# puzzlepaint/camera_calibration

Measured on AMD Instinct MI355X. Metric: M observations/sec per LM iteration, higher is better.
Workload: dtype f64

## Files before the change

camera_calibration_amd/build.py:

```python
from __future__ import annotations

import os
import shutil
import subprocess
import sys

HERE = os.path.dirname(os.path.abspath(__file__))
CSRC = os.path.join(HERE, "csrc")
LIB = os.path.join(HERE, "libcalib_ba_hip.so")
SOURCES = ["cba_api.hip", "cba_setup.hip", "cba_passes.hip", "cba_solve.hip", "cba_posefirst.hip", "cba_gridfirst.hip", "cba_oneshot.hip", "cba_report.hip", "cba_compare.hip", "cba_undistort.hip", "cba_features.hip",
           "kernels_project.hip", "kernels_fd.hip", "kernels_obs.hip", "kernels_update.hip", "kernels_linalg.hip", "kernels_ldlt.hip", "kernels_ldlt_dist.hip", "kernels_backsolve.hip", "kernels_fit.hip", "gridfirst_plan.hip", "kernels_gridfirst.hip", "kernels_report.hip", "kernels_compare.hip", "kernels_undistort.hip", "kernels_features.hip", "cba_localize.hip", "kernels_localize.hip", "cba_localize_images.hip", "kernels_localize_images.hip", "cba_parametric.hip", "kernels_parametric.hip", "cba_stereo.hip", "kernels_stereo.hip", "kernels_stereo_post.hip"]
HEADERS = ["cba_internal.h", "hip_buf.h", "cba_problem.h", "cba_model.h", "model.hip.h", "obs_device.hip.h", "block_device.hip.h", "localize_device.hip.h", "gridfirst_plan.h", "linalg_internal.h", "ldlt_dataflow.hip.h", os.path.join("..", "..", "include", "cba.h")]
PUBLIC_HEADERS = [os.path.join("..", "..", "include", "cba_undistort.h"), os.path.join("..", "..", "include", "cba_features.h"),
                  os.path.join("..", "..", "include", "cba_stereo.h"), os.path.join("..", "..", "include", "cba_stereo_post.h"),
                  os.path.join("..", "..", "include", "cba_diagnostics.h")]
FLAGS = ["--offload-arch=gfx950", "-O3", "-std=c++17", "-fPIC", "-munsafe-fp-atomics", "-Wall", "-Wno-unused-function", "-Wno-unused-value", "-Wno-unused-result",
         "-mllvm", "-amdgpu-mfma-vgpr-form"]


def _hipcc() -> str:
    for cand in (shutil.which("hipcc"), "/opt/rocm/bin/hipcc"):
        if cand and os.path.exists(cand):
            return cand
    raise RuntimeError("hipcc not found")


FLAGS_STAMP = os.path.join(HERE, ".build_flags")
# ... 222 lines not shown
```

camera_calibration_amd/csrc/cba_api.hip:

```cpp
#include <algorithm>
#include <cmath>
#include <cstdlib>
#include <cstring>
#include <memory>

#include "cba_problem.h"
#include "../../include/cba_diagnostics.h"

namespace cba {

static thread_local std::string g_error;
void set_error(const std::string& msg) { g_error = msg; }

struct GpermView { int* v[kMaxCameras] = {}; };
static GpermView gperm_view(const cba_problem* p) {
  GpermView g;
  for (int c = 0; c < kMaxCameras; ++c) g.v[c] = p->gperm[c];
  return g;
}

static int enqueue_candidate_cost(cba_problem* p, int cand, const int* guard) {
  CBA_TRY(launch_apply_update(p->L, p->cams, p->st[p->cur], p->x, p->st[cand], p->pose_slot, gperm_view(p).v, p->stream));
  CBA_TRY(residual_pass(p, cand, guard));
  return launch_reduce_costs(p->out.cost_ref, p->out.cost_test, nullptr, p->obs.n, p->red_partials, p->red8, p->stream);
// ... 51 lines not shown
  setenv("GPU_MAX_HW_QUEUES", "8", 0);
  CBA_TRY(select_device(config->device, "cba_create: "));
  std::unique_ptr<cba_problem, decltype(&cba_destroy)> p(new cba_problem(), &cba_destroy);
  p->cfg = *config;
  p->cams.assign(config->cameras, config->cameras + config->n_cameras);
  p->cfg.cameras = p->cams.data();
  p->device = config->device;
  make_layout(p->cfg, p->L);
  if (p->L.total_dof <= 0) { set_error("empty problem"); return CBA_ERR_ARG; }
  CBA_TRY(make_main_stream(&p->stream));
  CBA_TRY(choose_elimination_order(p.get(), config));
  CBA_TRY(alloc_pass_buffers(p.get()));
  CBA_TRY(alloc_system(p.get()));
  CBA_TRY(alloc_reduce_buffer(p.get(), config));
  CBA_TRY(setup_gf_sharding(p.get()));
  CBA_TRY(alloc_ldlt_workspace(p.get()));
  *out = p.release();
  return CBA_OK;
}

void cba_destroy(cba_problem* p) {
  if (!p) return;
  hipSetDevice(p->device);
  if (p->stream) hipStreamSynchronize(p->stream);
  delete p;
}

int cba_set_observations(cba_problem* p, int64_t n, const float* xy, const int32_t* point_index,
                         const int32_t* image_index, const int32_t* camera_index, const double* last_projection) {
  if (!p || n < 0 || (n > 0 && (!xy || !point_index || !image_index || !camera_index))) { set_error("cba_set_observations: bad argument"); return CBA_ERR_ARG; }
// ... 408 lines not shown
  for (int i = 0; i < 3; ++i) out[i] = v[i];
  return CBA_OK;
}
int cba_debug_straggler_stats(cba_problem* p, int64_t out[5]) {
  if (!p || !out || !p->slow.count) { set_error("cba_debug_straggler_stats: bad argument"); return CBA_ERR_ARG; }
  int v[kSlowCounters];
  CBA_HIP(hipSetDevice(p->device));
  CBA_HIP(hipStreamSynchronize(p->stream));
  CBA_TRY(p->slow.count.download(v, kSlowCounters));
  out[0] = 0;
  out[1] = v[kSlowListCount] < p->slow.cap ? v[kSlowListCount] : p->slow.cap;
  out[2] = v[kSlowStatPeriod1]; out[3] = v[kSlowStatPeriodN]; out[4] = v[kSlowStatFullBudget];
  return CBA_OK;
}

}
```

camera_calibration_amd/csrc/cba_internal.h:

```cpp
#pragma once
#include <hip/hip_runtime.h>
#include <stdint.h>

#include <chrono>
#include <string>
#include <type_traits>
#include <vector>

#include "../../include/cba.h"
#include "../../include/cba_features.h"
#include "gridfirst_plan.h"
#include "hip_buf.h"
#include "model.hip.h"

namespace cba {

class Event {
 public:
  Event() = default;
  Event(Event&& o) noexcept : e_(o.e_) { o.e_ = nullptr; }
  Event& operator=(Event&& o) noexcept {
    if (this != &o) { reset(); e_ = o.e_; o.e_ = nullptr; }
    return *this;
  }
// ... 150 lines not shown
                      const double* det_scale, int points_separate, hipStream_t s);
int launch_accumulate_points(const PassArgs& a, const Layout& L, const std::vector<cba_camera>& cams, const Observations& obs,
                             const PassOutputs& out, const SystemView& sys, const double* det_scale, hipStream_t s);
int launch_det_scale(const PassArgs& a, const PassOutputs& out, DetMode& det, hipStream_t s);
int launch_det_convert(double* p, size_t n, const double* det_scale, hipStream_t s);
int launch_accumulate_strips(const PassArgs& a, const Layout& L, const Observations& obs, const PassOutputs& out, CellSort& cell,
                             const SystemView& sys, const double* det_scale, hipStream_t s);
int launch_accumulate_cells(const PassArgs& a, const std::vector<cba_camera>& cams, const PassOutputs& out, CellSort& cell,
                            const SystemView& sys, int rig_row_first, const double* det_scale, hipStream_t s);
int launch_exclusive_scan(const int* count, int n, int* start, hipStream_t s);
int launch_reduce_costs(const double* ref, const double* test, const uint8_t* flags, int64_t n, double* partials,
                        double* out8, hipStream_t s);
int launch_apply_update(const Layout& L, const std::vector<cba_camera>& cams, const DevState& in, const double* x,
                        DevState& out, const int* pose_slot, int* const* gperm, hipStream_t s);
int launch_update_direction_grid(const double* in, const double* x, int G, double* out, hipStream_t s);
int launch_fit_pass(bool jac, int gw, int gh, const double* grid, const double* tang, int64_t n, const double* gp,
                    const double* dirs, double* cost_vec, double* rec, int* keys, int* status, hipStream_t s);
int launch_fit_accumulate(int gw, int gh, int64_t n, const double* rec, const int* keys, DevBuf<int>& count, int* start, DevBuf<int>& fill,
                          int* order, double* H, int ld, double* b, hipStream_t s);
int launch_fit_set_rhs(double* S, int ld, const double* b, int n, hipStream_t s);
int launch_fit_diag_sum(const double* H, int ld, int n, double* out, hipStream_t s);

int launch_direction_image(const CamDev* cam_dev, int model, int W, int H, double* dirs, uint8_t* ok, uint8_t* rgb, hipStream_t s,
                           bool use_stage = true);
struct SiteGrid {
  int side4;
  int bw, bh;
  const int* start;
  const int* order;
  const int* xy;
// ... 264 lines not shown
```

camera_calibration_amd/csrc/cba_passes.hip:

```cpp
#include "cba_problem.h"

namespace cba {

int timer_begin(cba_problem* p, int which, hipStream_t s) {
  KernelTimer& t = p->timers[which];
  if (t.used == (int)t.spans.size()) {
    KernelTimer::Span sp;
    CBA_TRY(sp.e0.create()); CBA_TRY(sp.e1.create());
    t.spans.push_back(std::move(sp));
  }
  CBA_HIP(hipEventRecord(t.spans[t.used].e0, s ? s : p->stream));
  return CBA_OK;
}
int timer_end(cba_problem* p, int which, double flops, double bytes, int launches, hipStream_t s) {
  KernelTimer& t = p->timers[which];
  CBA_HIP(hipEventRecord(t.spans[t.used].e1, s ? s : p->stream));
  t.used += 1;
  t.flops += flops; t.bytes += bytes; t.launches += launches;
  return CBA_OK;
}
int timers_collect(cba_problem* p) {
  for (KernelTimer& t : p->timers) {
    for (int i = 0; i < t.used; ++i) {
      CBA_HIP(hipEventSynchronize(t.spans[i].e1));
// ... 63 lines not shown
  CBA_HIP(hipEventRecord(p->ev_aux2, p->stream));
  CBA_HIP(hipStreamWaitEvent(aux, p->ev_aux2, 0));
  CBA_TRY(launch_base_project_slow(as, p->model_mask, p->out,  false, p->slow, aux));
  CBA_TRY(launch_fd_tasks(as, p->model_mask, L.localize_only, p->out, p->fd, kFdSideList, aux));
  CBA_HIP(hipEventRecord(p->ev_aux1, aux));
  CBA_TRY(timer_begin(p, kTimerFd));
  CBA_TRY(launch_fd_tasks(a, p->model_mask, L.localize_only, p->out, p->fd, kFdMainList, p->stream));
  CBA_TRY(timer_end(p, kTimerFd, 0, 0, 1));
  CBA_HIP(hipStreamWaitEvent(clr, p->ev_aux2, 0));
  CBA_TRY(p->sys.Dblk.zero_async(clr));
  CBA_TRY(p->sys.bblk.zero_async(clr));
  if (L.eliminate_points)
    CBA_TRY(p->sys.B.zero_async(clr));
  else
    CBA_TRY(p->sys.B.zero_async((size_t)(p->sys.Kpad - L.block_dof) * p->sys.n_pad, clr, (size_t)L.block_dof * p->sys.n_pad));
  CBA_TRY(p->sys.Hdd.zero_async(clr));
  CBA_TRY(p->sys.bd.zero_async(clr));
  if (p->gf.S0) CBA_TRY(p->gf.S0.zero_async(clr));
  CBA_HIP(hipEventRecord(p->ev_clear, clr));
  CBA_HIP(hipStreamWaitEvent(p->stream, p->ev_aux1, 0));
  CBA_HIP(hipStreamWaitEvent(p->stream, p->ev_clear, 0));
  a.skip = nullptr;
  const bool side = !L.localize_only;
  CBA_TRY(launch_assemble(a, L, p->st[w], p->out, p->slow, p->stream));
  double t0 = now_s();
  CBA_TRY(timer_begin(p, kTimerAccumulate));
  SystemView T = p->sys.view();
  const double* det = p->cfg.deterministic ? (const double*)p->det.scale : nullptr;
  if (det) CBA_TRY(launch_det_scale(a, p->out, p->det, p->stream));
  const int points_separate = (!L.eliminate_points && p->obs.pt_start) ? 1 : 0;
  if (p->gf.S0) {
// ... 5 lines not shown
    CBA_HIP(hipStreamWaitEvent(aux, p->ev_aux0, 0));
    CBA_TRY(launch_accumulate_cells(a, p->cams, p->out, p->cell, T, (!L.eliminate_points && L.rig_in_state) ? L.first_camera_tr_rig - L.block_dof : -1,
                                    det, aux));
    if (p->gridfirst) CBA_TRY(gridfirst_pass_activity(p, a, aux));
    CBA_HIP(hipEventRecord(p->ev_aux1, aux));
  }
  if (points_separate)
    CBA_TRY(launch_accumulate_points(a, L, p->cams, p->obs, p->out, T, det, p->stream));
  if (!L.eliminate_points)
    CBA_TRY(launch_accumulate_strips(a, L, p->obs, p->out, p->cell, T, det, p->stream));
  CBA_TRY(launch_accumulate(a, L, p->out, p->cell, T, det, points_separate, p->stream));
  if (side) CBA_HIP(hipStreamWaitEvent(p->stream, p->ev_aux1, 0));
  if (det) {
    CBA_TRY(launch_det_convert(p->sys.Dblk, nb * bs * bs, det, p->stream));
    CBA_TRY(launch_det_convert(p->sys.bblk, nb * bs, det + 1, p->stream));
    CBA_TRY(launch_det_convert(p->sys.Hdd, (size_t)L.dense_dof * p->sys.n_pad, det, p->stream));
    CBA_TRY(launch_det_convert(p->sys.bd, (size_t)p->sys.n_pad, det + 1, p->stream));
    CBA_TRY(launch_det_convert(p->sys.B, (size_t)L.block_dof * p->sys.n_pad, det, p->stream));
    if (p->gf.S0) CBA_TRY(launch_det_convert(p->gf.S0, p->gf.S0.size(), det, p->stream));
  }
  CBA_TRY(timer_end(p, kTimerAccumulate, 0, 0, 1));
  if (t_acc) *t_acc += now_s() - t0;
  CBA_TRY(p->gridfirst ? gridfirst_pass_end(p) : posefirst_pass_end(p));
  p->have_system = true;
  return CBA_OK;
}

}
```

camera_calibration_amd/csrc/cba_problem.h:

```cpp
#pragma once
#include <cmath>

#include "cba_internal.h"

using namespace cba;

struct KernelTimer {
  struct Span { Event e0, e1; };
  std::vector<Span> spans;
  int used = 0;
  double seconds = 0, flops = 0, bytes = 0;
  int launches = 0;
};
enum Timer {
  kTimerProduct,
  kTimerFactor,
  kTimerAccumulate,
  kTimerFd,
  kTimerFactorGemm,
  kTimerJacobianPass,
  kTimerSolve,
  kTimerCost,
  kNumTimers
};
// ... 19 lines not shown
  PinnedBuf<unsigned long long> kmask_host;
  double update_flops = 0;
  DevBuf<int> tile_list; PinnedBuf<int> tile_list_host; bool tile_list_valid = false; unsigned tile_list_age = 0;
  int tile_list_entries = 0;
  bool tile_list_dirty = false;
};

struct GfShardState {
  GfShared shared;
  DevBuf<int> shared_col;
  int rank = 0, world = 1, img0 = 0, max_local = 0;
  std::vector<int> counts, offsets;
  DevBuf<double> gDblk, gbblk, gB;
  DevBuf<double> gsend, grecv; int64_t gblk = 0;
};
#pragma GCC visibility pop

struct cba_problem {
  cba_config cfg{};
  std::vector<cba_camera> cams;
  Layout L{};
  int device = 0;
  hipStream_t stream = nullptr;
  bool have_obs = false, have_state = false, have_system = false;
  int model_mask = 0;
  Observations obs;
  PassOutputs out;
  StragglerSplit slow;
  FdWork fd;
  CellSort cell;
  DetMode det;
  DevState st[2];
  int cur = 0;
  DevBuf<double> itg;
  DevBuf<double> tangents[kMaxCameras];
  DevBuf<CamDev> cams_dev[2];
  std::vector<int> pose_slot_host; DevBuf<int> pose_slot;
  Event ev_aux0, ev_aux1, ev_aux2, ev_clear;
  DevBuf<int> gperm[kMaxCameras];
  std::vector<int> dense_perm_host;
  DevBuf<double> red_partials, red8;
  NormalSystem sys;
  double* P = nullptr; DevBuf<double> P_own;
  DevBuf<double> P2;
  int64_t P_cap = 0;
  DevBuf<double> x, scal;
  DevBuf<int> status;
  LdltWorkspace ldlt;
  KernelTimer timers[kNumTimers];
  double last_lambda = 0;
  PinnedBuf<double> pin_status;
  PinnedBuf<double> pin_cost;
  double last_x0 = 0;
  bool gridfirst = false;
  bool gf_sharded = false;
  PoseFirstState pf;
  GridFirstState gf;
// ... 15 lines not shown
      if (cx < 0 || cy < 0 || cx >= cm.grid_w || cy >= cm.grid_h) continue;
      fn(cx, cy);
    }
}
inline int common_slabs(const unsigned long long* a, const unsigned long long* b, int words) {
  int n = 0;
  for (int w = 0; w < words; ++w) n += __builtin_popcountll(a[w] & b[w]);
  return n;
}

void make_layout(const cba_config& cfg, Layout& L);
int check_config(const cba_config* config);
int choose_elimination_order(cba_problem* p, const cba_config* config);
int alloc_pass_buffers(cba_problem* p);
int alloc_system(cba_problem* p);
int alloc_reduce_buffer(cba_problem* p, const cba_config* config);
int alloc_ldlt_workspace(cba_problem* p);
void order_imagesets(cba_problem* p, int64_t n, const float* xy, const int32_t* point_index, const int32_t* image_index,
                     const int32_t* camera_index, std::vector<int>& order);

int timer_begin(cba_problem* p, int which, hipStream_t s = nullptr);
int timer_end(cba_problem* p, int which, double flops, double bytes, int launches, hipStream_t s = nullptr);
int timers_collect(cba_problem* p);
int allreduce(cba_problem* p, double* dev, int64_t count);
int residual_pass(cba_problem* p, int which, const int* guard = nullptr);
int jacobian_pass_and_accumulate(cba_problem* p, double* t_acc);

int solve_enqueue(cba_problem* p, double lambda);
int solve_finish(cba_problem* p);
int solve_system(cba_problem* p, double lambda);
// ... 21 lines not shown
```

camera_calibration_amd/csrc/cba_setup.hip:

```cpp
#include <algorithm>
#include <map>
#include <mutex>

#include "cba_problem.h"

namespace cba {

void make_layout(const cba_config& cfg, Layout& L) {
  L.n_cameras = cfg.n_cameras; L.n_images = cfg.n_images; L.n_points = cfg.n_points;
  L.localize_only = cfg.localize_only ? 1 : 0;
  L.eliminate_points = cfg.eliminate_points ? 1 : 0;
  const int N = cfg.n_images, C = cfg.n_cameras, P = cfg.n_points;
  L.rig_in_state = C > 1;
  const int rig_dof = L.rig_in_state ? 6 * C : 0;
  L.first_rig_tr_global = L.eliminate_points ? 3 * P : 0;
  L.first_camera_tr_rig = L.first_rig_tr_global + 6 * N;
  L.first_points = L.eliminate_points ? 0 : L.first_camera_tr_rig + rig_dof;
  L.first_intrinsics = L.eliminate_points ? (L.first_camera_tr_rig + rig_dof) : (L.first_points + 3 * P);
  if (L.eliminate_points) { L.block_size = 3; L.n_blocks = P; } else { L.block_size = 6; L.n_blocks = N; }
  L.block_dof = L.block_size * L.n_blocks;
  int off = L.first_intrinsics;
  for (int c = 0; c < C; ++c) {
    L.intr_offset[c] = off - L.block_dof;
    off += unknowns_per_point(cfg.cameras[c].model_type) * cfg.cameras[c].grid_w * cfg.cameras[c].grid_h;
// ... 76 lines not shown
  if (o->factor_tail_rows > 0) w.tail_rows = o->factor_tail_rows;
  w.back_dataflow = o->back_substitution == 0;
}

static int alloc_state(cba_problem* p, DevState& s) {
  CBA_TRY(s.rig_tr_global.alloc(7 * (size_t)p->L.n_images));
  CBA_TRY(s.camera_tr_rig.alloc(7 * (size_t)p->L.n_cameras));
  CBA_TRY(s.points.alloc(3 * (size_t)p->L.n_points));
  for (int c = 0; c < p->L.n_cameras; ++c) {
    size_t G = (size_t)p->cams[c].grid_w * p->cams[c].grid_h;
    CBA_TRY(s.grids[c].alloc(doubles_per_point(p->cams[c].model_type) * G));
  }
  return CBA_OK;
}

static int build_grid_order(cba_problem* p) {
  const Layout& L = p->L;
  p->dense_perm_host.resize(L.dense_dof);
  for (int i = 0; i < L.dense_dof; ++i) p->dense_perm_host[i] = i;
  if (L.localize_only) return CBA_OK;
  for (int c = 0; c < L.n_cameras; ++c) {
    const int gw = p->cams[c].grid_w, gh = p->cams[c].grid_h;
    const int per = unknowns_per_point(p->cams[c].model_type);
    const int tile = per == 2 ? 8 : 5;
    std::vector<int> perm((size_t)gw * gh);
    int rank = 0;
    if (p->gridfirst) perm = p->gf.plan.gperm[c];
    else
    for (int ty = 0; ty < gh; ty += tile)
      for (int tx = 0; tx < gw; tx += tile)
        for (int y = ty; y < std::min(gh, ty + tile); ++y)
          for (int x = tx; x < std::min(gw, tx + tile); ++x) perm[x + (size_t)y * gw] = rank++;
    CBA_TRY(p->gperm[c].assign(perm));
    for (size_t g = 0; g < perm.size(); ++g)
      for (int d = 0; d < per; ++d)
        p->dense_perm_host[L.intr_offset[c] + per * g + d] = L.intr_offset[c] + per * perm[g] + d;
  }
  return CBA_OK;
}

static int upload_camdevs(cba_problem* p, int which) {
  std::vector<CamDev> h(p->L.n_cameras);
  for (int c = 0; c < p->L.n_cameras; ++c)
    h[c] = make_camdev(p->cams[c], p->st[which].grids[c], p->tangents[c], p->L.intr_offset[c], p->gperm[c]);
  CBA_TRY(p->cams_dev[which].upload_async(h.data(), h.size(), p->stream));
  CBA_HIP(hipStreamSynchronize(p->stream));
  return CBA_OK;
}

int check_config(const cba_config* config) {
  if (!config || !config->cameras || config->n_cameras < 1 || config->n_cameras > kMaxCameras ||
      config->n_images < 0 || config->n_points < 0 || !(config->numerical_diff_delta > 0)) {
// ... 102 lines not shown
  CBA_TRY(p->det.bits.alloc(2)); CBA_TRY(p->det.scale.alloc(2));
  CBA_TRY(p->fd.redo_count.alloc_zero(4));
  CBA_TRY(p->red_partials.alloc(256 * 8));
  CBA_TRY(p->red8.alloc(16));
  return CBA_OK;
}

int alloc_system(cba_problem* p) {
  const Layout& L = p->L;
  padded_dims(L.dense_dof, &p->sys.n_pad, &p->sys.n_fact);
  p->sys.Kpad = round_up(L.block_dof > 0 ? L.block_dof : 1, 48);
  const size_t bs = L.block_size, nb = L.n_blocks;
  CBA_TRY(p->sys.Dblk.alloc(nb * bs * bs));
  CBA_TRY(p->sys.bblk.alloc(nb * bs));
  CBA_TRY(p->sys.B.alloc((size_t)p->sys.Kpad * p->sys.n_pad));
  CBA_TRY(p->sys.Hdd.alloc((size_t)p->sys.n_pad * p->sys.n_pad));
  CBA_TRY(p->sys.bd.alloc((size_t)p->sys.n_pad));
  CBA_TRY(p->gridfirst ? alloc_gridfirst_system(p) : alloc_posefirst_system(p));
  CBA_TRY(p->x.alloc_zero((size_t)L.block_dof + p->sys.n_pad));
  CBA_TRY(p->scal.alloc(16));
  CBA_TRY(p->status.alloc(2));
  CBA_TRY(p->pin_status.alloc(4));
  CBA_TRY(p->pin_cost.alloc(16));
  return CBA_OK;
}

int alloc_reduce_buffer(cba_problem* p, const cba_config* config) {
  if (!config->allreduce) return CBA_OK;
  int64_t need = p->gf_sharded ? p->sh.shared.doubles : packed_upper_doubles(p->sys.n_pad);
  if (config->distributed_solve) {
    need = (int64_t)ldlt_dist_buffer_doubles(p->sys.n_pad, config->world_size);
// ... 47 lines not shown
```

camera_calibration_amd/csrc/kernels_update.hip:

```cpp
#include "block_device.hip.h"
#include "obs_device.hip.h"

namespace cba {

constexpr int kRedBlocks = 256;
__global__ void __launch_bounds__(256) k_reduce_costs_partial(const double* __restrict__ ref, const double* __restrict__ test,
                                                              const uint8_t* __restrict__ flags, int64_t n,
                                                              double* __restrict__ partials) {
  double acc[8] = {0, 0, 0, 0, 0, 0, 0, 0};
  for (int64_t i = (int64_t)blockIdx.x * 256 + threadIdx.x; i < n; i += (int64_t)kRedBlocks * 256) {
    double r = ref ? ref[i] : -1.0, t = test ? test[i] : -1.0;
    if (r >= 0) { acc[0] += r; acc[5] += 1; }
    if (t >= 0) { acc[1] += t; acc[6] += 1; }
    if (r >= 0 && t >= 0) { acc[2] += r; acc[3] += t; acc[4] += 1; }
    if (flags && flags[i] == 1) acc[7] += 1;
  }
  __shared__ double sh[8][256];
  block_reduce_256(acc, sh, SumOp());
  if (threadIdx.x < 8) partials[blockIdx.x * 8 + threadIdx.x] = sh[threadIdx.x][0];
}
int launch_reduce_costs(const double* ref, const double* test, const uint8_t* flags, int64_t n, double* partials,
                        double* out8, hipStream_t s) {
  hipLaunchKernelGGL(k_reduce_costs_partial, dim3(kRedBlocks), dim3(256), 0, s, ref, test, flags, n, partials);
  hipLaunchKernelGGL((k_fold_partials<8, kRedBlocks, SumOp>), dim3(1), dim3(64), 0, s, partials, out8);
// ... 73 lines not shown
    hipLaunchKernelGGL(k_update_grid, dim3((G + 255) / 256), dim3(256), 0, s, in.grids[c],
                       x + (L.localize_only ? 0 : L.block_dof + L.intr_offset[c]), G, per, L.localize_only ? 0 : 1,
                       gperm ? gperm[c] : nullptr, out.grids[c]);
  }
  CBA_HIP(hipGetLastError());
  return CBA_OK;
}

int launch_update_direction_grid(const double* in, const double* x, int G, double* out, hipStream_t s) {
  if (G == 0) return CBA_OK;
  hipLaunchKernelGGL(k_update_grid, dim3((G + 255) / 256), dim3(256), 0, s, in, x, G, 2, 1, (const int*)nullptr, out);
  CBA_HIP(hipGetLastError());
  return CBA_OK;
}

}
```

camera_calibration_amd/engine.py:

```python
from __future__ import annotations

import ctypes as C
import os
from dataclasses import dataclass
from typing import Callable, List, Optional, Sequence

import numpy as np

from .problem import CENTRAL_GENERIC, Camera, Problem, State

_HERE = os.path.dirname(os.path.abspath(__file__))
LIB_PATH = os.environ.get("CBA_HIP_LIB") or os.path.join(_HERE, "libcalib_ba_hip.so")


class EngineError(RuntimeError):
    pass


class CbaCamera(C.Structure):
    _fields_ = [("model_type", C.c_int32), ("width", C.c_int32), ("height", C.c_int32),
                ("calib_min_x", C.c_int32), ("calib_min_y", C.c_int32),
                ("calib_max_x", C.c_int32), ("calib_max_y", C.c_int32),
                ("grid_w", C.c_int32), ("grid_h", C.c_int32)]

# ... 202 lines not shown
    "cba_remap_apply_device": (_I, [_VP, _I32, _I32, _I32, _I32, _VP, _VP, C.c_uint8, _VP]),
}


class CbaStereoOptions(C.Structure):
    _fields_ = [("context_radius", C.c_int32), ("iterations", C.c_int32), ("min_depth", C.c_float), ("max_depth", C.c_float),
                ("max_normal_2d_length", C.c_float), ("cost_threshold", C.c_float), ("angle_threshold", C.c_float),
                ("lr_consistency_factor_threshold", C.c_float), ("seed", C.c_uint64)]


_I8P, _SOPT = C.POINTER(C.c_int8), C.POINTER(CbaStereoOptions)
DIAGNOSTICS_PROTOTYPES = {
    "cba_debug_straggler_stats": (_I, [_VP, _I64P]),
    "cba_debug_gridfirst_tile_list_query": (_I64, [_I32, _I32, _I32, C.POINTER(C.c_uint64), _I32, _I32, _I32P, _I64]),
    "cba_debug_gridfirst_tile_list": (_I64, [_VP, _I32P, _I64, _I32P]),
}
STEREO_PROTOTYPES = {
    "cba_stereo_create": (_I, [_I32, _I32, _I32, _I32, _F32P, C.c_float, C.c_float, C.c_float, C.c_float, _I32, _I32, _F32P, _F32P, _I32,
                               C.POINTER(_VP)]),
    "cba_stereo_destroy": (None, [_VP]),
    "cba_stereo_set_images": (_I, [_VP, _U8, _U8]),
    "cba_stereo_set_pose": (_I, [_VP, _F32P]),
    "cba_stereo_match": (_I, [_VP, _SOPT]),
    "cba_stereo_get_state": (_I, [_VP, _F32P, _I8P, _F32P]),
    "cba_stereo_set_state": (_I, [_VP, _F32P, _I8P, _F32P]),
    "cba_stereo_run_stage": (_I, [_VP, _SOPT, _I32, _I32]),
    "cba_stereo_cost": (_I, [_VP, _SOPT, _F32P, _I8P, _F32P]),
    "cba_stereo_filter": (_I, [_VP, _SOPT, _F32P, _F32P]),
}
STEREO_INIT, STEREO_MUTATION, STEREO_PROPAGATION, STEREO_REFINEMENT = 0, 1, 2, 3
# ... 26 lines not shown
def load() -> C.CDLL:
    global _lib
    if _lib is not None:
        return _lib
    os.environ.setdefault("GPU_MAX_HW_QUEUES", "8")
    try:
        import torch
    except Exception:
        pass
    if not os.path.exists(LIB_PATH):
        raise EngineError(f"{LIB_PATH} is missing -- run `python -c 'import __graft_entry__ as g; g.build()'`; "
                          "the engine has no CPU fallback")
    L = C.CDLL(LIB_PATH)
    for name, (restype, argtypes) in {**PROTOTYPES, **UNDISTORT_PROTOTYPES, **STEREO_PROTOTYPES, **STEREO_POST_PROTOTYPES,
                                      **DIAGNOSTICS_PROTOTYPES}.items():
        fn = getattr(L, name)
        fn.restype, fn.argtypes = restype, argtypes
    _lib = L
    return L


def gridfirst_plan(cameras: Sequence[Camera], n_images: int, n_points: int, strips: int = 0, single_tile_tasks: bool = False) -> dict:
    L = load()
    cams = (CbaCamera * len(cameras))(*[_cam_struct(c) for c in cameras])

    def q(what, dtype):
        n = L.cba_gridfirst_plan_query(cams, len(cameras), n_images, n_points, strips, int(single_tile_tasks), what, None, 0)
        if n < 0:
            _check(int(n), "cba_gridfirst_plan_query")
        out = np.zeros(int(n) // np.dtype(dtype).itemsize, dtype=dtype)
        if n:
# ... 19 lines not shown

def gridfirst_tile_list_query(mode: int, masks: np.ndarray, n_slabs: int, allow_parts: bool) -> np.ndarray:
    L = load()
    m = np.ascontiguousarray(masks, dtype=np.uint64)
    assert m.ndim == 2
    mp = m.ctypes.data_as(C.POINTER(C.c_uint64))
    n = int(L.cba_debug_gridfirst_tile_list_query(int(mode), m.shape[0], m.shape[1], mp, int(n_slabs), int(bool(allow_parts)), None, 0))
    if n < 0:
        _check(n, "cba_debug_gridfirst_tile_list_query")
    out = np.zeros((n, 4), dtype=np.int32)
    if n:
        got = int(L.cba_debug_gridfirst_tile_list_query(int(mode), m.shape[0], m.shape[1], mp, int(n_slabs), int(bool(allow_parts)),
                                                        out.ctypes.data_as(_I32P), n))
        assert got == n
    return out


def prepare(device: int = 0) -> None:
    _check(load().cba_prepare_device(int(device)), "cba_prepare_device")


def _check(rc: int, what: str) -> None:
    if rc != 0:
        msg = load().cba_last_error()
        raise EngineError(f"{what} failed with code {rc}: {msg.decode() if msg else ''}")


def _dp(a: np.ndarray):
    assert a.dtype == np.float64 and a.flags.c_contiguous
    return a.ctypes.data_as(C.POINTER(C.c_double))
# ... 157 lines not shown
    def straggler_stats(self) -> dict:
        out = (C.c_int64 * 5)()
        _check(self.L.cba_debug_straggler_stats(self._h, out), "cba_debug_straggler_stats")
        return dict(zip(("predicted", "listed", "period_1", "period_2_or_more", "full_budget"), (int(v) for v in out)))

    def gridfirst_tile_list(self):
        info = (C.c_int32 * 4)()
        n = int(self.L.cba_debug_gridfirst_tile_list(self._h, None, 0, info))
        if n < 0:
            _check(n, "cba_debug_gridfirst_tile_list")
        out = np.zeros((n, 4), dtype=np.int32)
        if n:
            assert int(self.L.cba_debug_gridfirst_tile_list(self._h, out.ctypes.data_as(_I32P), n, info)) == n
        return out, dict(valid=int(info[0]), age=int(info[1]), dirty=int(info[2]), n_slabs=int(info[3]))

    def debug_accumulate(self) -> float:
        cost = C.c_double(0)
        _check(self.L.cba_debug_accumulate(self._h, C.byref(cost)), "cba_debug_accumulate")
        return cost.value

    def debug_solve(self, lam: float) -> np.ndarray:
        _check(self.L.cba_debug_solve(self._h, lam), "cba_debug_solve")
        return self.dump(DUMP_X)

    def debug_apply_update(self, x: np.ndarray) -> None:
        x = np.ascontiguousarray(x, dtype=np.float64)
        assert x.size == self.problem.total_dof
        _check(self.L.cba_debug_apply_update(self._h, _dp(x)), "cba_debug_apply_update")

    def dump(self, what: int) -> np.ndarray:
# ... 605 lines not shown
```

include/cba_diagnostics.h:

```cpp
#ifndef CBA_DIAGNOSTICS_H
#define CBA_DIAGNOSTICS_H

#include "cba.h"

#ifdef __cplusplus
extern "C" {
#endif

int cba_debug_straggler_stats(cba_problem* p, int64_t out[5]);

int64_t cba_debug_gridfirst_tile_list_query(int32_t mode, int32_t nt, int32_t words, const uint64_t* mask_words, int32_t n_slabs,
                                            int32_t allow_parts, int32_t* entries, int64_t capacity_entries);
int64_t cba_debug_gridfirst_tile_list(cba_problem* p, int32_t* entries, int64_t capacity_entries, int32_t info[4]);

#ifdef __cplusplus
}
#endif

#endif
```

Baseline: 36.32.

## Clear and convert only the structurally written segments of the dense Hessian block

Precomputes on the host the sparsity pattern of the dense-dense Hessian block (pose/rig rows, point rows, grid neighbourhoods within a 7x7 stencil, shared sharded columns) as row segments. Each iteration, a segmented kernel zeroes only those entries, and the same list drives the deterministic fixed-point-to-double conversion, instead of a full n_pad^2 memset and convert. The list is used only when it covers at most about half of the upper triangle. This relies on the pattern being exact, and the buffer is now zero-initialised at allocation so untouched entries stay zero. Debug entry points to inspect or disable the list are added.

```diff
diff --git a/camera_calibration_amd/build.py b/camera_calibration_amd/build.py
--- a/camera_calibration_amd/build.py
+++ b/camera_calibration_amd/build.py
@@ -9,8 +9,8 @@
 CSRC = os.path.join(HERE, "csrc")
 LIB = os.path.join(HERE, "libcalib_ba_hip.so")
 SOURCES = ["cba_api.hip", "cba_setup.hip", "cba_passes.hip", "cba_solve.hip", "cba_posefirst.hip", "cba_gridfirst.hip", "cba_oneshot.hip", "cba_report.hip", "cba_compare.hip", "cba_undistort.hip", "cba_features.hip",
-           "kernels_project.hip", "kernels_fd.hip", "kernels_obs.hip", "kernels_update.hip", "kernels_linalg.hip", "kernels_ldlt.hip", "kernels_ldlt_dist.hip", "kernels_backsolve.hip", "kernels_fit.hip", "gridfirst_plan.hip", "kernels_gridfirst.hip", "kernels_report.hip", "kernels_compare.hip", "kernels_undistort.hip", "kernels_features.hip", "cba_localize.hip", "kernels_localize.hip", "cba_localize_images.hip", "kernels_localize_images.hip", "cba_parametric.hip", "kernels_parametric.hip", "cba_stereo.hip", "kernels_stereo.hip", "kernels_stereo_post.hip"]
-HEADERS = ["cba_internal.h", "hip_buf.h", "cba_problem.h", "cba_model.h", "model.hip.h", "obs_device.hip.h", "block_device.hip.h", "localize_device.hip.h", "gridfirst_plan.h", "linalg_internal.h", "ldlt_dataflow.hip.h", os.path.join("..", "..", "include", "cba.h")]
+           "kernels_project.hip", "kernels_fd.hip", "kernels_obs.hip", "kernels_update.hip", "kernels_linalg.hip", "kernels_ldlt.hip", "kernels_ldlt_dist.hip", "kernels_backsolve.hip", "kernels_fit.hip", "gridfirst_plan.hip", "hdd_clear_list.hip", "kernels_gridfirst.hip", "kernels_report.hip", "kernels_compare.hip", "kernels_undistort.hip", "kernels_features.hip", "cba_localize.hip", "kernels_localize.hip", "cba_localize_images.hip", "kernels_localize_images.hip", "cba_parametric.hip", "kernels_parametric.hip", "cba_stereo.hip", "kernels_stereo.hip", "kernels_stereo_post.hip"]
+HEADERS = ["cba_internal.h", "hip_buf.h", "cba_problem.h", "cba_model.h", "model.hip.h", "obs_device.hip.h", "block_device.hip.h", "localize_device.hip.h", "gridfirst_plan.h", "hdd_clear_list.h", "linalg_internal.h", "ldlt_dataflow.hip.h", os.path.join("..", "..", "include", "cba.h")]
 PUBLIC_HEADERS = [os.path.join("..", "..", "include", "cba_undistort.h"), os.path.join("..", "..", "include", "cba_features.h"),
                   os.path.join("..", "..", "include", "cba_stereo.h"), os.path.join("..", "..", "include", "cba_stereo_post.h"),
                   os.path.join("..", "..", "include", "cba_diagnostics.h")]
diff --git a/camera_calibration_amd/csrc/cba_api.hip b/camera_calibration_amd/csrc/cba_api.hip
--- a/camera_calibration_amd/csrc/cba_api.hip
+++ b/camera_calibration_amd/csrc/cba_api.hip
@@ -89,6 +89,8 @@
   CBA_TRY(alloc_system(p.get()));
   CBA_TRY(alloc_reduce_buffer(p.get(), config));
   CBA_TRY(setup_gf_sharding(p.get()));
+  hdd_clear_list_host(p.get());
+  CBA_TRY(upload_hdd_clear_list(p.get()));
   CBA_TRY(alloc_ldlt_workspace(p.get()));
   *out = p.release();
   return CBA_OK;
@@ -527,4 +529,40 @@
   return CBA_OK;
 }
 
-}
+static int64_t give_hdd_clear_list(const cba_problem* p, int32_t* segments, int64_t capacity_segments, int64_t info[4]) {
+  const int64_t n = (int64_t)p->hddc.segs.size();
+  if (info) {
+    int n_pad = 0, n_fact = 0;
+    padded_dims(p->L.dense_dof, &n_pad, &n_fact);
+    info[0] = n_pad; info[1] = p->L.dense_dof; info[2] = p->hddc.entries; info[3] = p->hddc.selective ? 1 : 0;
+  }
+  if (segments && capacity_segments >= n)
+    for (int64_t i = 0; i < n; ++i) { segments[3 * i] = p->hddc.segs[i].row; segments[3 * i + 1] = p->hddc.segs[i].col; segments[3 * i + 2] = p->hddc.segs[i].len; }
+  return n;
+}
+int64_t cba_debug_hdd_clear_list_query(const cba_config* config, int32_t* segments, int64_t capacity_segments, int64_t info[4]) {
+  CBA_TRY(check_config(config));
+  cba_problem tmp;
+  tmp.cfg = *config;
+  tmp.cams.assign(config->cameras, config->cameras + config->n_cameras);
+  tmp.cfg.cameras = tmp.cams.data();
+  make_layout(tmp.cfg, tmp.L);
+  if (tmp.L.total_dof <= 0) { set_error("empty problem"); return CBA_ERR_ARG; }
+  CBA_TRY(choose_elimination_order(&tmp, config));
+  grid_order_host(&tmp);
+  hdd_clear_list_host(&tmp);
+  return give_hdd_clear_list(&tmp, segments, capacity_segments, info);
+}
+int64_t cba_debug_hdd_clear_list(cba_problem* p, int32_t* segments, int64_t capacity_segments, int64_t info[4]) {
+  if (!p) { set_error("cba_debug_hdd_clear_list: bad argument"); return CBA_ERR_ARG; }
+  const int64_t n = give_hdd_clear_list(p, segments, capacity_segments, info);
+  if (info) info[3] = (p->hddc.selective && !p->hddc.force_full) ? 1 : 0;
+  return n;
+}
+int cba_debug_set_hdd_full_clear(cba_problem* p, int32_t on) {
+  if (!p) { set_error("cba_debug_set_hdd_full_clear: bad argument"); return CBA_ERR_ARG; }
+  p->hddc.force_full = on != 0;
+  return CBA_OK;
+}
+
+}
diff --git a/camera_calibration_amd/csrc/cba_internal.h b/camera_calibration_amd/csrc/cba_internal.h
--- a/camera_calibration_amd/csrc/cba_internal.h
+++ b/camera_calibration_amd/csrc/cba_internal.h
@@ -188,6 +188,9 @@
 int launch_apply_update(const Layout& L, const std::vector<cba_camera>& cams, const DevState& in, const double* x,
                         DevState& out, const int* pose_slot, int* const* gperm, hipStream_t s);
 int launch_update_direction_grid(const double* in, const double* x, int G, double* out, hipStream_t s);
+struct HddPiece { long long off; int len, pad; };
+constexpr int kHddPieceMax = 1024;
+int launch_hdd_segments(double* H, const HddPiece* pieces, int n_pieces, const double* det_scale, hipStream_t s);
 int launch_fit_pass(bool jac, int gw, int gh, const double* grid, const double* tang, int64_t n, const double* gp,
                     const double* dirs, double* cost_vec, double* rec, int* keys, int* status, hipStream_t s);
 int launch_fit_accumulate(int gw, int gh, int64_t n, const double* rec, const int* keys, DevBuf<int>& count, int* start, DevBuf<int>& fill,
diff --git a/camera_calibration_amd/csrc/cba_passes.hip b/camera_calibration_amd/csrc/cba_passes.hip
--- a/camera_calibration_amd/csrc/cba_passes.hip
+++ b/camera_calibration_amd/csrc/cba_passes.hip
@@ -101,7 +101,9 @@
     CBA_TRY(p->sys.B.zero_async(clr));
   else
     CBA_TRY(p->sys.B.zero_async((size_t)(p->sys.Kpad - L.block_dof) * p->sys.n_pad, clr, (size_t)L.block_dof * p->sys.n_pad));
-  CBA_TRY(p->sys.Hdd.zero_async(clr));
+  const bool hdd_list = p->hddc.selective && !p->hddc.force_full;
+  if (hdd_list) CBA_TRY(launch_hdd_segments(p->sys.Hdd, p->hddc.pieces, p->hddc.n_pieces, nullptr, clr));
+  else CBA_TRY(p->sys.Hdd.zero_async(clr));
   CBA_TRY(p->sys.bd.zero_async(clr));
   if (p->gf.S0) CBA_TRY(p->gf.S0.zero_async(clr));
   CBA_HIP(hipEventRecord(p->ev_clear, clr));
@@ -137,7 +139,8 @@
   if (det) {
     CBA_TRY(launch_det_convert(p->sys.Dblk, nb * bs * bs, det, p->stream));
     CBA_TRY(launch_det_convert(p->sys.bblk, nb * bs, det + 1, p->stream));
-    CBA_TRY(launch_det_convert(p->sys.Hdd, (size_t)L.dense_dof * p->sys.n_pad, det, p->stream));
+    if (hdd_list) CBA_TRY(launch_hdd_segments(p->sys.Hdd, p->hddc.pieces, p->hddc.n_pieces, det, p->stream));
+    else CBA_TRY(launch_det_convert(p->sys.Hdd, (size_t)L.dense_dof * p->sys.n_pad, det, p->stream));
     CBA_TRY(launch_det_convert(p->sys.bd, (size_t)p->sys.n_pad, det + 1, p->stream));
     CBA_TRY(launch_det_convert(p->sys.B, (size_t)L.block_dof * p->sys.n_pad, det, p->stream));
     if (p->gf.S0) CBA_TRY(launch_det_convert(p->gf.S0, p->gf.S0.size(), det, p->stream));
diff --git a/camera_calibration_amd/csrc/cba_problem.h b/camera_calibration_amd/csrc/cba_problem.h
--- a/camera_calibration_amd/csrc/cba_problem.h
+++ b/camera_calibration_amd/csrc/cba_problem.h
@@ -2,6 +2,7 @@
 #include <cmath>
 
 #include "cba_internal.h"
+#include "hdd_clear_list.h"
 
 using namespace cba;
 
@@ -57,6 +58,12 @@
   DevBuf<double> gDblk, gbblk, gB;
   DevBuf<double> gsend, grecv; int64_t gblk = 0;
 };
+struct HddClearState {
+  std::vector<HddSeg> segs; int64_t entries = 0;
+  DevBuf<HddPiece> pieces; int n_pieces = 0;
+  bool selective = false;
+  bool force_full = false;
+};
 #pragma GCC visibility pop
 
 struct cba_problem {
@@ -81,9 +88,11 @@
   std::vector<int> pose_slot_host; DevBuf<int> pose_slot;
   Event ev_aux0, ev_aux1, ev_aux2, ev_clear;
   DevBuf<int> gperm[kMaxCameras];
+  std::vector<int> gperm_host[kMaxCameras];
   std::vector<int> dense_perm_host;
   DevBuf<double> red_partials, red8;
   NormalSystem sys;
+  HddClearState hddc;
   double* P = nullptr; DevBuf<double> P_own;
   DevBuf<double> P2;
   int64_t P_cap = 0;
@@ -129,6 +138,9 @@
 int choose_elimination_order(cba_problem* p, const cba_config* config);
 int alloc_pass_buffers(cba_problem* p);
 int alloc_system(cba_problem* p);
+void grid_order_host(cba_problem* p);
+void hdd_clear_list_host(cba_problem* p);
+int upload_hdd_clear_list(cba_problem* p);
 int alloc_reduce_buffer(cba_problem* p, const cba_config* config);
 int alloc_ldlt_workspace(cba_problem* p);
 void order_imagesets(cba_problem* p, int64_t n, const float* xy, const int32_t* point_index, const int32_t* image_index,
diff --git a/camera_calibration_amd/csrc/cba_setup.hip b/camera_calibration_amd/csrc/cba_setup.hip
--- a/camera_calibration_amd/csrc/cba_setup.hip
+++ b/camera_calibration_amd/csrc/cba_setup.hip
@@ -114,11 +114,11 @@
   return CBA_OK;
 }
 
-static int build_grid_order(cba_problem* p) {
+void grid_order_host(cba_problem* p) {
   const Layout& L = p->L;
   p->dense_perm_host.resize(L.dense_dof);
   for (int i = 0; i < L.dense_dof; ++i) p->dense_perm_host[i] = i;
-  if (L.localize_only) return CBA_OK;
+  if (L.localize_only) return;
   for (int c = 0; c < L.n_cameras; ++c) {
     const int gw = p->cams[c].grid_w, gh = p->cams[c].grid_h;
     const int per = unknowns_per_point(p->cams[c].model_type);
@@ -131,11 +131,45 @@
       for (int tx = 0; tx < gw; tx += tile)
         for (int y = ty; y < std::min(gh, ty + tile); ++y)
           for (int x = tx; x < std::min(gw, tx + tile); ++x) perm[x + (size_t)y * gw] = rank++;
-    CBA_TRY(p->gperm[c].assign(perm));
     for (size_t g = 0; g < perm.size(); ++g)
       for (int d = 0; d < per; ++d)
         p->dense_perm_host[L.intr_offset[c] + per * g + d] = L.intr_offset[c] + per * perm[g] + d;
-  }
+    p->gperm_host[c] = std::move(perm);
+  }
+}
+static int build_grid_order(cba_problem* p) {
+  grid_order_host(p);
+  if (p->L.localize_only) return CBA_OK;
+  for (int c = 0; c < p->L.n_cameras; ++c) CBA_TRY(p->gperm[c].assign(p->gperm_host[c]));
+  return CBA_OK;
+}
+
+void hdd_clear_list_host(cba_problem* p) {
+  const Layout& L = p->L;
+  HddWriteSet w;
+  w.cams = p->cams.data(); w.n_cameras = L.n_cameras; w.n_images = L.n_images; w.n_points = L.n_points;
+  w.eliminate_points = L.eliminate_points; w.localize_only = L.localize_only;
+  for (int c = 0; c < L.n_cameras; ++c) w.gperm[c] = p->gperm_host[c].empty() ? nullptr : p->gperm_host[c].data();
+  w.point_rows_in_strips = p->gridfirst && !p->gf_sharded;
+  std::vector<int> col;
+  if (p->gf_sharded) {
+    col.resize(p->sh.shared.ref_col.size());
+    for (size_t k = 0; k < col.size(); ++k) col[k] = p->dense_perm_host[p->sh.shared.ref_col[k]];
+    w.shared = &p->sh.shared; w.shared_col = col.data();
+  }
+  p->hddc.entries = hdd_write_segments(w, &p->hddc.segs);
+  p->hddc.selective = 4 * p->hddc.entries <= (int64_t)L.dense_dof * (L.dense_dof + 1);
+}
+int upload_hdd_clear_list(cba_problem* p) {
+  const int64_t ld = p->sys.n_pad;
+  std::vector<HddPiece> pieces;
+  for (const HddSeg& s : p->hddc.segs) {
+    if (s.row < 0 || s.col < s.row || s.len <= 0 || s.col + s.len > p->L.dense_dof) { set_error("cba_create: bad segment of H_dd"); return CBA_ERR_STATE; }
+    for (int c = 0; c < s.len; c += kHddPieceMax) pieces.push_back(HddPiece{s.row * ld + s.col + c, std::min(kHddPieceMax, s.len - c), 0});
+  }
+  if (pieces.size() > 0x7fffff00u) p->hddc.selective = false;
+  p->hddc.n_pieces = p->hddc.selective ? (int)pieces.size() : 0;
+  if (p->hddc.selective) CBA_TRY(p->hddc.pieces.assign(pieces));
   return CBA_OK;
 }
 
@@ -268,7 +302,7 @@
   CBA_TRY(p->sys.Dblk.alloc(nb * bs * bs));
   CBA_TRY(p->sys.bblk.alloc(nb * bs));
   CBA_TRY(p->sys.B.alloc((size_t)p->sys.Kpad * p->sys.n_pad));
-  CBA_TRY(p->sys.Hdd.alloc((size_t)p->sys.n_pad * p->sys.n_pad));
+  CBA_TRY(p->sys.Hdd.alloc_zero((size_t)p->sys.n_pad * p->sys.n_pad));
   CBA_TRY(p->sys.bd.alloc((size_t)p->sys.n_pad));
   CBA_TRY(p->gridfirst ? alloc_gridfirst_system(p) : alloc_posefirst_system(p));
   CBA_TRY(p->x.alloc_zero((size_t)L.block_dof + p->sys.n_pad));
diff --git a/camera_calibration_amd/csrc/hdd_clear_list.h b/camera_calibration_amd/csrc/hdd_clear_list.h
--- /dev/null
+++ b/camera_calibration_amd/csrc/hdd_clear_list.h
@@ -0,0 +1,25 @@
+#pragma once
+#include <stdint.h>
+
+#include <vector>
+
+#include "../../include/cba.h"
+#include "gridfirst_plan.h"
+
+namespace cba {
+
+struct HddSeg { int row, col, len; };
+
+struct HddWriteSet {
+  const cba_camera* cams = nullptr;
+  int n_cameras = 0, n_images = 0, n_points = 0;
+  int eliminate_points = 0, localize_only = 0;
+  const int* gperm[16] = {};
+  int point_rows_in_strips = 0;
+  const GfShared* shared = nullptr;
+  const int* shared_col = nullptr;
+};
+
+int64_t hdd_write_segments(const HddWriteSet& in, std::vector<HddSeg>* out);
+
+}
diff --git a/camera_calibration_amd/csrc/hdd_clear_list.hip b/camera_calibration_amd/csrc/hdd_clear_list.hip
--- /dev/null
+++ b/camera_calibration_amd/csrc/hdd_clear_list.hip
@@ -0,0 +1,83 @@
+#include "hdd_clear_list.h"
+
+#include <algorithm>
+
+namespace cba {
+
+namespace {
+
+struct Ival { int row, c0, c1; };
+
+inline int ppg_of(const cba_camera& c) { return c.model_type == CBA_CENTRAL_GENERIC ? 2 : 5; }
+
+}
+
+int64_t hdd_write_segments(const HddWriteSet& in, std::vector<HddSeg>* out) {
+  const int C = in.n_cameras, N = in.n_images, P = in.n_points;
+  const int rig_dof = C > 1 ? 6 * C : 0;
+  const int rig0 = in.eliminate_points ? 6 * N : 0;
+  const int g0 = rig0 + rig_dof + (in.eliminate_points ? 0 : 3 * P);
+  std::vector<int> first_col(C + 1, g0);
+  for (int c = 0; c < C; ++c)
+    first_col[c + 1] = first_col[c] + (in.localize_only ? 0 : ppg_of(in.cams[c]) * in.cams[c].grid_w * in.cams[c].grid_h);
+  const int dd = first_col[C];
+  std::vector<Ival> iv;
+  auto add = [&](int row, int c0, int c1) {
+    c0 = std::max(c0, row);
+    if (c0 < c1) iv.push_back(Ival{row, c0, c1});
+  };
+  if (in.eliminate_points)
+    for (int r = 0; r < 6 * N; ++r) { add(r, r, r - r % 6 + 6); add(r, rig0, dd); }
+  for (int r = rig0; r < rig0 + rig_dof; ++r) add(r, r, dd);
+  if (!in.eliminate_points) {
+    const bool over_grid = !in.point_rows_in_strips || in.shared;
+    for (int r = rig_dof; r < g0; ++r) {
+      add(r, r, r - (r - rig_dof) % 3 + 3);
+      if (over_grid) add(r, g0, dd);
+    }
+  }
+  if (!in.localize_only) {
+    for (int c = 0; c < C; ++c) {
+      const int gw = in.cams[c].grid_w, gh = in.cams[c].grid_h, per = ppg_of(in.cams[c]);
+      const int* perm = in.gperm[c];
+      auto col_of = [&](int x, int y) { const int s = x + y * gw; return first_col[c] + per * (perm ? perm[s] : s); };
+      for (int y = 0; y < gh; ++y)
+        for (int x = 0; x < gw; ++x) {
+          const int u = col_of(x, y);
+          for (int y2 = std::max(0, y - 3); y2 <= std::min(gh - 1, y + 3); ++y2)
+            for (int x2 = std::max(0, x - 3); x2 <= std::min(gw - 1, x + 3); ++x2) {
+              const int v = col_of(x2, y2);
+              if (v < u) continue;
+              for (int d = 0; d < per; ++d) add(u + d, v, v + per);
+            }
+        }
+    }
+    if (in.shared) {
+      const GfShared& sh = *in.shared;
+      for (int c = 0; c < sh.n_cameras; ++c) {
+        const int n = sh.cam_pos[c + 1] - sh.cam_pos[c];
+        for (int i = 0; i < n; ++i)
+          for (int k = 0; k < sh.width[c] && i + k < n; ++k) {
+            const int u = in.shared_col[sh.cam_pos[c] + i], v = in.shared_col[sh.cam_pos[c] + i + k];
+            add(std::min(u, v), std::max(u, v), std::max(u, v) + 1);
+          }
+      }
+    }
+  }
+  std::sort(iv.begin(), iv.end(), [](const Ival& a, const Ival& b) { return a.row != b.row ? a.row < b.row : a.c0 < b.c0; });
+  out->clear();
+  int64_t entries = 0;
+  for (const Ival& v : iv) {
+    if (!out->empty() && out->back().row == v.row && v.c0 <= out->back().col + out->back().len) {
+      const int end = std::max(out->back().col + out->back().len, v.c1);
+      entries += end - (out->back().col + out->back().len);
+      out->back().len = end - out->back().col;
+    } else {
+      out->push_back(HddSeg{v.row, v.c0, v.c1 - v.c0});
+      entries += v.c1 - v.c0;
+    }
+  }
+  return entries;
+}
+
+}
diff --git a/camera_calibration_amd/csrc/kernels_update.hip b/camera_calibration_amd/csrc/kernels_update.hip
--- a/camera_calibration_amd/csrc/kernels_update.hip
+++ b/camera_calibration_amd/csrc/kernels_update.hip
@@ -1,3 +1,5 @@
+#include <algorithm>
+
 #include "block_device.hip.h"
 #include "obs_device.hip.h"
 
@@ -111,4 +113,36 @@
   return CBA_OK;
 }
 
+template <bool CONVERT>
+__global__ void __launch_bounds__(256) k_hdd_segments(double* __restrict__ H, const HddPiece* __restrict__ pieces, int n_pieces,
+                                                      const double* __restrict__ det_scale) {
+  const double inv = CONVERT ? 1.0 / *det_scale : 0.0;
+  auto put = [&](double* q) { *q = CONVERT ? (double)(*reinterpret_cast<const long long*>(q)) * inv : 0.0; };
+  const int sub = threadIdx.x & 15;
+  for (int i = blockIdx.x * 16 + (threadIdx.x >> 4); i < n_pieces; i += gridDim.x * 16) {
+    const HddPiece pc = pieces[i];
+    double* q = H + pc.off;
+    const int head = (int)(pc.off & 1), pairs = (pc.len - head) >> 1;
+    if (head && sub == 0) put(q);
+    if (sub == 15 && ((pc.len - head) & 1)) put(q + pc.len - 1);
+    double2* q2 = reinterpret_cast<double2*>(q + head);
+    for (int j = sub; j < pairs; j += 16) {
+      if (CONVERT) {
+        const longlong2 v = *reinterpret_cast<const longlong2*>(q2 + j);
+        q2[j] = make_double2((double)v.x * inv, (double)v.y * inv);
+      } else {
+        q2[j] = make_double2(0.0, 0.0);
+      }
+    }
+  }
 }
+int launch_hdd_segments(double* H, const HddPiece* pieces, int n_pieces, const double* det_scale, hipStream_t s) {
+  if (n_pieces <= 0) return CBA_OK;
+  const unsigned blocks = (unsigned)std::min((n_pieces + 15) / 16, 4096);
+  if (det_scale) hipLaunchKernelGGL(k_hdd_segments<true>, dim3(blocks), dim3(256), 0, s, H, pieces, n_pieces, det_scale);
+  else hipLaunchKernelGGL(k_hdd_segments<false>, dim3(blocks), dim3(256), 0, s, H, pieces, n_pieces, det_scale);
+  CBA_HIP(hipGetLastError());
+  return CBA_OK;
+}
+
+}
diff --git a/camera_calibration_amd/engine.py b/camera_calibration_amd/engine.py
--- a/camera_calibration_amd/engine.py
+++ b/camera_calibration_amd/engine.py
@@ -240,6 +240,9 @@
     "cba_debug_straggler_stats": (_I, [_VP, _I64P]),
     "cba_debug_gridfirst_tile_list_query": (_I64, [_I32, _I32, _I32, C.POINTER(C.c_uint64), _I32, _I32, _I32P, _I64]),
     "cba_debug_gridfirst_tile_list": (_I64, [_VP, _I32P, _I64, _I32P]),
+    "cba_debug_hdd_clear_list_query": (_I64, [_CFG, _I32P, _I64, _I64P]),
+    "cba_debug_hdd_clear_list": (_I64, [_VP, _I32P, _I64, _I64P]),
+    "cba_debug_set_hdd_full_clear": (_I, [_VP, _I32]),
 }
 STEREO_PROTOTYPES = {
     "cba_stereo_create": (_I, [_I32, _I32, _I32, _I32, _F32P, C.c_float, C.c_float, C.c_float, C.c_float, _I32, _I32, _F32P, _F32P, _I32,
@@ -296,7 +299,11 @@
     L = C.CDLL(LIB_PATH)
     for name, (restype, argtypes) in {**PROTOTYPES, **UNDISTORT_PROTOTYPES, **STEREO_PROTOTYPES, **STEREO_POST_PROTOTYPES,
                                       **DIAGNOSTICS_PROTOTYPES}.items():
-        fn = getattr(L, name)
+        fn = getattr(L, name, None)
+        if fn is None and name in DIAGNOSTICS_PROTOTYPES and os.environ.get("CBA_HIP_LIB"):
+            continue
+        if fn is None:
+            raise AttributeError(f"{LIB_PATH} does not export {name}")
         fn.restype, fn.argtypes = restype, argtypes
     _lib = L
     return L
@@ -346,6 +353,30 @@
                                                         out.ctypes.data_as(_I32P), n))
         assert got == n
     return out
+
+
+HDD_CLEAR_INFO = ("n_pad", "dense_dof", "entries", "selective")
+
+
+def _hdd_clear_list(call, what: str):
+    info = (C.c_int64 * 4)()
+    n = int(call(None, 0, info))
+    if n < 0:
+        _check(n, what)
+    out = np.zeros((n, 3), dtype=np.int32)
+    if n:
+        assert int(call(out.ctypes.data_as(_I32P), n, info)) == n
+    return out, {k: int(v) for k, v in zip(HDD_CLEAR_INFO, info)}
+
+
+def hdd_clear_list_query(problem: Problem, elimination: int = 0, grid_strips: int = 0):
+    L = load()
+    cams = (CbaCamera * problem.n_cameras)(*[_cam_struct(c) for c in problem.cameras])
+    cfg = CbaConfig(problem.n_cameras, cams, problem.n_images, problem.n_points, problem.fd_delta,
+                    int(problem.localize_only), int(problem.eliminate_points), 0, ALLREDUCE_FN(0), None, 0, None, 0, 0,
+                    0, 0, 1, COLLECTIVE_FN(0), None, CbaSolverOptions(0, 0, int(elimination), int(grid_strips), 0))
+    return _hdd_clear_list(lambda seg, cap, info: L.cba_debug_hdd_clear_list_query(C.byref(cfg), seg, cap, info),
+                           "cba_debug_hdd_clear_list_query")
 
 
 def prepare(device: int = 0) -> None:
@@ -533,6 +564,12 @@
             assert int(self.L.cba_debug_gridfirst_tile_list(self._h, out.ctypes.data_as(_I32P), n, info)) == n
         return out, dict(valid=int(info[0]), age=int(info[1]), dirty=int(info[2]), n_slabs=int(info[3]))
 
+    def hdd_clear_list(self):
+        return _hdd_clear_list(lambda seg, cap, info: self.L.cba_debug_hdd_clear_list(self._h, seg, cap, info), "cba_debug_hdd_clear_list")
+
+    def set_hdd_full_clear(self, on: bool) -> None:
+        _check(self.L.cba_debug_set_hdd_full_clear(self._h, int(bool(on))), "cba_debug_set_hdd_full_clear")
+
     def debug_accumulate(self) -> float:
         cost = C.c_double(0)
         _check(self.L.cba_debug_accumulate(self._h, C.byref(cost)), "cba_debug_accumulate")
diff --git a/include/cba_diagnostics.h b/include/cba_diagnostics.h
--- a/include/cba_diagnostics.h
+++ b/include/cba_diagnostics.h
@@ -13,6 +13,10 @@
                                             int32_t allow_parts, int32_t* entries, int64_t capacity_entries);
 int64_t cba_debug_gridfirst_tile_list(cba_problem* p, int32_t* entries, int64_t capacity_entries, int32_t info[4]);
 
+int64_t cba_debug_hdd_clear_list_query(const cba_config* config, int32_t* segments, int64_t capacity_segments, int64_t info[4]);
+int64_t cba_debug_hdd_clear_list(cba_problem* p, int32_t* segments, int64_t capacity_segments, int64_t info[4]);
+int cba_debug_set_hdd_full_clear(cba_problem* p, int32_t on);
+
 #ifdef __cplusplus
 }
 #endif
```

Measured after the change: 36.90 (median of 6 runs). +1.6%, better.
